# naman1618/Distributed-Inference-with-PyTorch-and-LiteLLM

Hardware: AMD Instinct MI355X
Metric: fine-tune tokens/sec (whole node) Llama-3.1-70B DDP at 1/2/4/8 MI355X (higher is better)
Workload: dtype bf16; 1 GPU; model=Llama-3.1-70B, global_batch=2, seq_len=2048, parallelism=dp1, finetune=lora r=16 alpha=32.0 on q,k,v,o,gate,up,down; frozen bf16 base, micro_batch=2, grad_accum=1, activation_checkpointing=False, optimizer=fused AdamW (HIP), grad clip 1.0, grad_reduce_dtype=bf16

## Files before the change

csrc/kernels/lora.hip:

```cpp
#include "bindings.h"
#include "common.h"
#include <stdlib.h>
#include <string.h>

namespace mx {

namespace {

typedef __bf16 lbf16x8_t __attribute__((ext_vector_type(8)));
typedef __attribute__((address_space(1))) const void* lgptr_t;
typedef __attribute__((address_space(3))) void* llptr_t;

__device__ __forceinline__ f32x4 lmfma(const u16x8& a, const u16x8& b, const f32x4& c) {
  return __builtin_amdgcn_mfma_f32_16x16x32_bf16(__builtin_bit_cast(lbf16x8_t, a), __builtin_bit_cast(lbf16x8_t, b),
                                                 c, 0, 0, 0);
}

constexpr int kRS = 68;
constexpr int kMaxTiles = 16384;

__device__ unsigned int g_xwt_cnt[kMaxTiles];
__device__ unsigned int g_xtg_cnt[kMaxTiles];

__device__ __forceinline__ bool arrive_last(unsigned int* cnt, int S, int* s_flag) {
  __threadfence();
  __syncthreads();
  if (threadIdx.x == 0) {
    const unsigned prev = atomicAdd(cnt, 1u);
    *s_flag = prev == (unsigned)(S - 1);
    if (*s_flag) *cnt = 0u;
  }
  __syncthreads();
  const bool last = *s_flag;
  if (last) __threadfence();
  return last;
}

__device__ __forceinline__ void st4_sc1(float* p, const float4& v) {
  __hip_atomic_store(p + 0, v.x, __ATOMIC_RELAXED, __HIP_MEMORY_SCOPE_AGENT);
  __hip_atomic_store(p + 1, v.y, __ATOMIC_RELAXED, __HIP_MEMORY_SCOPE_AGENT);
  __hip_atomic_store(p + 2, v.z, __ATOMIC_RELAXED, __HIP_MEMORY_SCOPE_AGENT);
  __hip_atomic_store(p + 3, v.w, __ATOMIC_RELAXED, __HIP_MEMORY_SCOPE_AGENT);
}
__device__ __forceinline__ float4 ld4_sc1(const float* p) {
  float* q = const_cast<float*>(p);
  return float4{__hip_atomic_load(q + 0, __ATOMIC_RELAXED, __HIP_MEMORY_SCOPE_AGENT),
                __hip_atomic_load(q + 1, __ATOMIC_RELAXED, __HIP_MEMORY_SCOPE_AGENT),
                __hip_atomic_load(q + 2, __ATOMIC_RELAXED, __HIP_MEMORY_SCOPE_AGENT),
                __hip_atomic_load(q + 3, __ATOMIC_RELAXED, __HIP_MEMORY_SCOPE_AGENT)};
}
__device__ __forceinline__ bool arrive_last_sc1(unsigned int* cnt, int S, int* s_flag) {
  asm volatile("s_waitcnt vmcnt(0)" ::: "memory");
  __syncthreads();
  if (threadIdx.x == 0) {
    const unsigned prev = __hip_atomic_fetch_add(cnt, 1u, __ATOMIC_RELAXED, __HIP_MEMORY_SCOPE_AGENT);
    const int last = prev == (unsigned)(S - 1);
    if (last) __hip_atomic_store(cnt, 0u, __ATOMIC_RELAXED, __HIP_MEMORY_SCOPE_AGENT);
    *s_flag = last;
  }
  __syncthreads();
  return *s_flag;
}

}

__global__ void __launch_bounds__(256, 1) lora_xwt_kernel(const uint16_t* __restrict__ X, int64_t ldx,
                                                          const uint16_t* __restrict__ V, int64_t ldv,
                                                          uint16_t* __restrict__ out, int64_t ldo,
                                                          float* __restrict__ ws, int M, int K, int S, float alpha,
                                                          int fused_red) {
  __shared__ __attribute__((aligned(16))) float red[4][64 * kRS];
  __shared__ int s_last;
  const int mtiles = M >> 6, mt = blockIdx.x, split = blockIdx.y;
  const int tid = threadIdx.x, lane = tid & 63, c = lane & 15, g = lane >> 4;
  const int w = __builtin_amdgcn_readfirstlane(tid >> 6);
  const int nb = K >> 6, nw = S * 4, gw = split * 4 + w;
  const int b0 = (int)((int64_t)gw * nb / nw), b1 = (int)((int64_t)(gw + 1) * nb / nw);
  const uint16_t* xp = X + (int64_t)(mt * 64 + c) * ldx + 16 * g;
  const uint16_t* vp = V + (int64_t)c * ldv + 16 * g;
  const int64_t xrb = 16 * ldx, vcb = 16 * ldv;

  f32x4 acc[4][4];
#pragma unroll
  for (int i = 0; i < 4; ++i)
// ... 155 lines not shown
#pragma unroll
    for (int j = 0; j < 4; ++j)
#pragma unroll
      for (int e = 0; e < 4; ++e) rw[(16 * i + 4 * g + e) * kRS + 16 * j + c] = acc[i][j][e];
  __syncthreads();
  float4 v[4];
#pragma unroll
  for (int q = 0; q < 4; ++q) {
    const int e4 = tid + 256 * q, row = e4 >> 4, col = (e4 & 15) * 4;
    float4 s = *reinterpret_cast<const float4*>(reinterpret_cast<const float*>(smem) + row * kRS + col);
#pragma unroll
    for (int ww = 1; ww < 4; ++ww) {
      const float4 t = *reinterpret_cast<const float4*>(reinterpret_cast<const float*>(smem + ww * WREG) +
                                                        row * kRS + col);
      s.x += t.x, s.y += t.y, s.z += t.z, s.w += t.w;
    }
    v[q] = s;
  }
  if (S > 1) {
    float* wp = ws + ((int64_t)split * mtiles + mt) * 4096;
    if (!fused_red) {
#pragma unroll
      for (int q = 0; q < 4; ++q) reinterpret_cast<float4*>(wp)[tid + 256 * q] = v[q];
      return;
    }
#pragma unroll
    for (int q = 0; q < 4; ++q) st4_sc1(wp + 4 * (tid + 256 * q), v[q]);
    if (!arrive_last_sc1(&g_xwt_cnt[mt], S, s_last)) return;
#pragma unroll
    for (int q = 0; q < 4; ++q) {
      float4 s = ld4_sc1(ws + (int64_t)mt * 4096 + 4 * (tid + 256 * q));
      for (int sp = 1; sp < S; ++sp) {
        const float4 t = ld4_sc1(ws + ((int64_t)sp * mtiles + mt) * 4096 + 4 * (tid + 256 * q));
        s.x += t.x, s.y += t.y, s.z += t.z, s.w += t.w;
      }
      v[q] = s;
    }
  }
#pragma unroll
  for (int q = 0; q < 4; ++q) {
    const int e4 = tid + 256 * q, row = e4 >> 4, col = (e4 & 15) * 4;
    uint2 o;
    o.x = pack_bf16x2(alpha * v[q].x, alpha * v[q].y);
    o.y = pack_bf16x2(alpha * v[q].z, alpha * v[q].w);
    *reinterpret_cast<uint2*>(out + (int64_t)(mt * 64 + row) * ldo + col) = o;
  }
}

__global__ void __launch_bounds__(256) lora_xwt_reduce_kernel(const float* __restrict__ ws, int S, int mtiles,
                                                              uint16_t* __restrict__ out, int64_t ldo, float alpha,
                                                              int qpw) {
  const int per = 4 / qpw;
  const int mt = blockIdx.x / per, tid = threadIdx.x;
  for (int q = (blockIdx.x % per) * qpw; q < (blockIdx.x % per + 1) * qpw; ++q) {
    const int e4 = tid + 256 * q, row = e4 >> 4, col = (e4 & 15) * 4;
    float4 s = reinterpret_cast<const float4*>(ws + (int64_t)mt * 4096)[e4];
    for (int sp = 1; sp < S; ++sp) {
      const float4 t = reinterpret_cast<const float4*>(ws + ((int64_t)sp * mtiles + mt) * 4096)[e4];
      s.x += t.x, s.y += t.y, s.z += t.z, s.w += t.w;
    }
    uint2 o;
    o.x = pack_bf16x2(alpha * s.x, alpha * s.y);
    o.y = pack_bf16x2(alpha * s.z, alpha * s.w);
    *reinterpret_cast<uint2*>(out + (int64_t)(mt * 64 + row) * ldo + col) = o;
  }
}

struct XtgProb {
  const uint16_t* X;
  const uint16_t* G;
  uint16_t* out;
  int64_t ldx, ldg, os_n, os_j;
  int Nx, jb0, JB, tile0;
};
constexpr int kMaxProb = 8;
struct XtgArgs {
  XtgProb p[kMaxProb];
  int np, T, S, ntiles;
  float alpha;
  int accumulate;
  int fused_red;
  int narrow3;
  int wt;
};

__device__ __forceinline__ int xsw(int row) { return (((row >> 1) & 1) << 2) | (((row >> 2) & 1) << 1); }

__global__ void __launch_bounds__(256, 1) lora_xtg_kernel(const XtgArgs a, float* __restrict__ ws) {
  constexpr int XB = 8192, STG = 16384, WREG = 2 * STG;
  __shared__ __attribute__((aligned(16))) char smem[4 * WREG];
  __shared__ int s_last;
  const int tid = threadIdx.x, lane = tid & 63, c = lane & 15, g = lane >> 4;
  const int w = __builtin_amdgcn_readfirstlane(tid >> 6);
  const int tile = a.wt ? blockIdx.x * 4 + w : blockIdx.x, split = blockIdx.y;
  if (a.wt && tile >= a.ntiles) return;
  XtgProb P = a.p[0];
#pragma unroll
  for (int i = 1; i < kMaxProb; ++i)
    if (i < a.np && tile >= a.p[i].tile0) P = a.p[i];
  const int n0 = (tile - P.tile0) * 64;
  const bool wide = P.JB > 1;
  const int JB = P.JB;
  const int qq = c >> 2, pp = c & 3;
  const int nblk = a.T >> 6, nw = a.wt ? a.S : a.S * 4, gw = a.wt ? split : split * 4 + w;
  const int b0 = (int)((int64_t)gw * nblk / nw), b1 = (int)((int64_t)(gw + 1) * nblk / nw);
  char* wreg = smem + w * WREG;
  const uint32_t wbase = lds_addr(wreg);

  const int xrow = lane >> 3, xch = (lane & 7) ^ xsw(lane >> 3);
  const uint16_t* xsrc = P.X + (int64_t)xrow * P.ldx + n0 + 8 * xch;
  const uint16_t* gsrc = wide ? P.G + (int64_t)xrow * P.ldg + 16 * P.jb0 + 8 * xch
                              : P.G + (int64_t)(lane >> 1) * P.ldg + 16 * P.jb0 + 8 * (lane & 1);
  auto issue = [&](int b, int s) {
    const int64_t t0 = (int64_t)b * 64;
    char* xs = wreg + s * STG;
#pragma unroll
    for (int q = 0; q < 8; ++q)
      __builtin_amdgcn_global_load_lds((lgptr_t)(xsrc + (t0 + 8 * q) * P.ldx), (llptr_t)(xs + q * 1024), 16, 0, 0);
    if (wide) {
#pragma unroll
      for (int q = 0; q < 8; ++q)
        __builtin_amdgcn_global_load_lds((lgptr_t)(gsrc + (t0 + 8 * q) * P.ldg), (llptr_t)(xs + XB + q * 1024), 16, 0,
                                         0);
    } else {
#pragma unroll
      for (int q = 0; q < 2; ++q)
        __builtin_amdgcn_global_load_lds((lgptr_t)(gsrc + (t0 + 32 * q) * P.ldg), (llptr_t)(xs + XB + q * 1024), 16,
                                         0, 0);
    }
  };
  const int fl = xsw(4 * g + qq);
  uint32_t xb[4];
#pragma unroll
  for (int i = 0; i < 4; ++i) xb[i] = wbase + (4 * g + qq) * 128 + 16 * ((2 * i + (pp >> 1)) ^ fl) + 8 * (pp & 1);
  const uint32_t gnb = wbase + XB + (4 * g + qq) * 32 + 8 * pp;

  f32x4 acc[4][4];
#pragma unroll
  for (int i = 0; i < 4; ++i)
#pragma unroll
    for (int j = 0; j < 4; ++j) acc[i][j] = f32x4{0.f, 0.f, 0.f, 0.f};

  auto block = [&](auto SC, int b) {
    constexpr int s = decltype(SC)::value;
    if (b + 1 < b1) {
      if (wide) asm volatile("s_waitcnt vmcnt(16)" ::: "memory");
      else asm volatile("s_waitcnt vmcnt(10)" ::: "memory");
    } else {
      asm volatile("s_waitcnt vmcnt(0)" ::: "memory");
    }
    u16x4 xr[2][2][4], gr[2][2][4];
#pragma unroll
    for (int ks = 0; ks < 2; ++ks)
#pragma unroll
      for (int h = 0; h < 2; ++h) {
#pragma unroll
        for (int i = 0; i < 4; ++i) xr[ks][h][i] = trd_off(xb[i], s * STG + (32 * ks + 16 * h) * 128);
        if (wide) {
#pragma unroll
          for (int j = 0; j < 4; ++j)
            if (j < JB) gr[ks][h][j] = trd_off(xb[j], s * STG + XB + (32 * ks + 16 * h) * 128);
        } else {
          gr[ks][h][0] = trd_off(gnb, s * STG + (32 * ks + 16 * h) * 32);
        }
      }
    lds_wait();
#pragma unroll
    for (int ks = 0; ks < 2; ++ks)
#pragma unroll
      for (int h = 0; h < 2; ++h) {
#pragma unroll
        for (int i = 0; i < 4; ++i) pin(xr[ks][h][i]);
#pragma unroll
        for (int j = 0; j < 4; ++j)
          if (j < JB) pin(gr[ks][h][j]);
      }
    if (b + 2 < b1) issue(b + 2, s);
#pragma unroll
    for (int ks = 0; ks < 2; ++ks) {
#pragma unroll
      for (int j = 0; j < 4; ++j) {
        if (j >= JB) continue;
        const u16x8 bf = u16x8{gr[ks][0][j][0], gr[ks][0][j][1], gr[ks][0][j][2], gr[ks][0][j][3],
                               gr[ks][1][j][0], gr[ks][1][j][1], gr[ks][1][j][2], gr[ks][1][j][3]};
#pragma unroll
        for (int i = 0; i < 4; ++i) {
          const u16x8 af = u16x8{xr[ks][0][i][0], xr[ks][0][i][1], xr[ks][0][i][2], xr[ks][0][i][3],
                                 xr[ks][1][i][0], xr[ks][1][i][1], xr[ks][1][i][2], xr[ks][1][i][3]};
          acc[i][j] = lmfma(af, bf, acc[i][j]);
        }
      }
    }
  };
  if (wide || !a.narrow3) {
    if (b0 < b1) issue(b0, 0);
    if (b0 + 1 < b1) issue(b0 + 1, 1);
    for (int b = b0; b < b1; b += 2) {
      block(std::integral_constant<int, 0>{}, b);
      if (b + 1 < b1) block(std::integral_constant<int, 1>{}, b + 1);
    }
  } else {
    constexpr int STN = XB + 2048;
    auto issue3 = [&](int b, int st) {
      const int64_t t0 = (int64_t)b * 64;
      char* xs = wreg + st * STN;
#pragma unroll
      for (int q = 0; q < 8; ++q)
        __builtin_amdgcn_global_load_lds((lgptr_t)(xsrc + (t0 + 8 * q) * P.ldx), (llptr_t)(xs + q * 1024), 16, 0, 0);
#pragma unroll
      for (int q = 0; q < 2; ++q)
        __builtin_amdgcn_global_load_lds((lgptr_t)(gsrc + (t0 + 32 * q) * P.ldg), (llptr_t)(xs + XB + q * 1024), 16,
                                         0, 0);
    };
    auto block3 = [&](auto SC, int b) {
      constexpr int st = decltype(SC)::value;
      if (b + 2 < b1) asm volatile("s_waitcnt vmcnt(20)" ::: "memory");
      else if (b + 1 < b1) asm volatile("s_waitcnt vmcnt(10)" ::: "memory");
      else asm volatile("s_waitcnt vmcnt(0)" ::: "memory");
      u16x4 xr[2][2][4], gr[2][2];
#pragma unroll
      for (int ks = 0; ks < 2; ++ks)
#pragma unroll
        for (int h = 0; h < 2; ++h) {
#pragma unroll
          for (int i = 0; i < 4; ++i) xr[ks][h][i] = trd_off(xb[i], st * STN + (32 * ks + 16 * h) * 128);
          gr[ks][h] = trd_off(gnb, st * STN + (32 * ks + 16 * h) * 32);
        }
      lds_wait();
#pragma unroll
      for (int ks = 0; ks < 2; ++ks)
#pragma unroll
        for (int h = 0; h < 2; ++h) {
#pragma unroll
          for (int i = 0; i < 4; ++i) pin(xr[ks][h][i]);
          pin(gr[ks][h]);
        }
      if (b + 3 < b1) issue3(b + 3, st);
#pragma unroll
      for (int ks = 0; ks < 2; ++ks) {
        const u16x8 bf = u16x8{gr[ks][0][0], gr[ks][0][1], gr[ks][0][2], gr[ks][0][3],
                               gr[ks][1][0], gr[ks][1][1], gr[ks][1][2], gr[ks][1][3]};
#pragma unroll
        for (int i = 0; i < 4; ++i) {
          const u16x8 af = u16x8{xr[ks][0][i][0], xr[ks][0][i][1], xr[ks][0][i][2], xr[ks][0][i][3],
                                 xr[ks][1][i][0], xr[ks][1][i][1], xr[ks][1][i][2], xr[ks][1][i][3]};
          acc[i][0] = lmfma(af, bf, acc[i][0]);
        }
      }
    };
    if (b0 < b1) issue3(b0, 0);
    if (b0 + 1 < b1) issue3(b0 + 1, 1);
    if (b0 + 2 < b1) issue3(b0 + 2, 2);
    for (int b = b0; b < b1; b += 3) {
      block3(std::integral_constant<int, 0>{}, b);
      if (b + 1 < b1) block3(std::integral_constant<int, 1>{}, b + 1);
      if (b + 2 < b1) block3(std::integral_constant<int, 2>{}, b + 2);
    }
  }
  float* rw = reinterpret_cast<float*>(wreg);
#pragma unroll
  for (int i = 0; i < 4; ++i)
#pragma unroll
    for (int j = 0; j < 4; ++j) {
      if (j >= JB) continue;
#pragma unroll
      for (int e = 0; e < 4; ++e) rw[(16 * i + 4 * g + e) * kRS + 16 * j + c] = acc[i][j][e];
    }
  if (a.wt) {
    asm volatile("s_waitcnt lgkmcnt(0)" ::: "memory");
    __builtin_amdgcn_wave_barrier();
    const int J = 16 * JB, nel = 64 * J;
    const bool jfast = P.os_j == 1;
    for (int e = lane; e < nel; e += 64) {
      const int n = jfast ? e / J : (e & 63), j = jfast ? e % J : (e >> 6);
      uint16_t* o = P.out + (int64_t)(n0 + n) * P.os_n + (int64_t)j * P.os_j;
      const float r = a.alpha * rw[n * kRS + j] + (a.accumulate ? bf2f(*o) : 0.f);
      *o = f2bf(r);
    }
    return;
  }
  __syncthreads();
  const int J = 16 * JB, nel = 64 * J;
  const bool jfast = P.os_j == 1;
  float v[16];
#pragma unroll
  for (int q = 0; q < 16; ++q) {
    const int e = tid + 256 * q;
    v[q] = 0.f;
    if (e < nel) {
      const int n = jfast ? e / J : (e & 63), j = jfast ? e % J : (e >> 6);
      float s = 0.f;
#pragma unroll
      for (int ww = 0; ww < 4; ++ww) s += reinterpret_cast<const float*>(smem + ww * WREG)[n * kRS + j];
      v[q] = s;
    }
  }
  if (a.S > 1) {
    float* wp = ws + ((int64_t)split * a.ntiles + tile) * 4096;
    if (!a.fused_red) {
#pragma unroll
      for (int q = 0; q < 16; ++q)
        if (tid + 256 * q < nel) wp[tid + 256 * q] = v[q];
      return;
    }
#pragma unroll
    for (int q = 0; q < 16; ++q)
      if (tid + 256 * q < nel) __hip_atomic_store(wp + tid + 256 * q, v[q], __ATOMIC_RELAXED, __HIP_MEMORY_SCOPE_AGENT);
    if (!arrive_last_sc1(&g_xtg_cnt[tile], a.S, &s_last)) return;
#pragma unroll
    for (int q = 0; q < 16; ++q) {
      const int e = tid + 256 * q;
      if (e < nel) {
        float s = __hip_atomic_load(ws + (int64_t)tile * 4096 + e, __ATOMIC_RELAXED, __HIP_MEMORY_SCOPE_AGENT);
        for (int sp = 1; sp < a.S; ++sp)
          s += __hip_atomic_load(ws + ((int64_t)sp * a.ntiles + tile) * 4096 + e, __ATOMIC_RELAXED,
                                 __HIP_MEMORY_SCOPE_AGENT);
        v[q] = s;
      }
    }
  }
#pragma unroll
  for (int q = 0; q < 16; ++q) {
    const int e = tid + 256 * q;
    if (e < nel) {
      const int n = jfast ? e / J : (e & 63), j = jfast ? e % J : (e >> 6);
      uint16_t* o = P.out + (int64_t)(n0 + n) * P.os_n + (int64_t)j * P.os_j;
      const float r = a.alpha * v[q] + (a.accumulate ? bf2f(*o) : 0.f);
      *o = f2bf(r);
    }
  }
}

__global__ void __launch_bounds__(256) lora_xtg_reduce_kernel(const XtgArgs a, const float* __restrict__ ws) {
  const int tile = blockIdx.x, tid = threadIdx.x;
  XtgProb P = a.p[0];
#pragma unroll
  for (int i = 1; i < kMaxProb; ++i)
    if (i < a.np && tile >= a.p[i].tile0) P = a.p[i];
  const int n0 = (tile - P.tile0) * 64, J = 16 * P.JB, nel = 64 * J;
  const bool jfast = P.os_j == 1;
  for (int e = tid; e < nel; e += 256) {
    float s = ws[(int64_t)tile * 4096 + e];
    for (int sp = 1; sp < a.S; ++sp) s += ws[((int64_t)sp * a.ntiles + tile) * 4096 + e];
    const int n = jfast ? e / J : (e & 63), j = jfast ? e % J : (e >> 6);
    uint16_t* o = P.out + (int64_t)(n0 + n) * P.os_n + (int64_t)j * P.os_j;
    *o = f2bf(a.alpha * s + (a.accumulate ? bf2f(*o) : 0.f));
  }
}

constexpr int kSlRow = 136;

__device__ __forceinline__ float sl_sigmoid(float x) { return __builtin_amdgcn_rcpf(1.f + __expf(-x)); }

template <bool BWD, int NRB, int RBW>
__global__ void __launch_bounds__(256) swiglu_lora_kernel(const uint16_t* __restrict__ gu,
                                                          const uint16_t* __restrict__ dm, uint16_t* __restrict__ out,
                                                          int64_t ldo, const uint16_t* __restrict__ V, int64_t ldv,
                                                          float* __restrict__ ws, int F, int CS) {
  constexpr int NP = BWD ? 2 : 1;
  constexpr int NC = 16 * NRB;
  __shared__ __attribute__((aligned(16))) uint16_t img[2][NP][RBW][16 * kSlRow];
  __shared__ __attribute__((aligned(16))) float red[4][16][NC + 4];
  const int rg = blockIdx.x, split = blockIdx.y, tid = threadIdx.x;
  const int lane = tid & 63, w = tid >> 6, r = lane & 15, gq = lane >> 4;
  const int row = tid >> 4, ch = tid & 15;
  const int tiles = F >> 7;
  const int t0 = (int)((int64_t)split * tiles / CS), t1 = (int)((int64_t)(split + 1) * tiles / CS);
  const int64_t tok = (int64_t)rg * 16 * RBW + row;
  const uint16_t* grow = gu + tok * (2 * (int64_t)F) + 8 * ch;
  const uint16_t* drow = dm + tok * (int64_t)F + 8 * ch;
  uint16_t* orow = out + tok * ldo + 8 * ch;
  const int64_t gstep = 16 * (2 * (int64_t)F), dstep = 16 * (int64_t)F, ostep = 16 * ldo;
  const uint16_t* vrow = V + (int64_t)r * ldv + 32 * w + 8 * gq;
  const int wofs = row * kSlRow + 8 * ch, rofs = r * kSlRow + 32 * w + 8 * gq;

  f32x4 acc[RBW][NRB];
#pragma unroll
  for (int i = 0; i < RBW; ++i)
#pragma unroll
    for (int b = 0; b < NRB; ++b) acc[i][b] = f32x4{0.f, 0.f, 0.f, 0.f};

  u16x8 g[RBW], u[RBW], d[RBW], vf[NP][NRB];
  auto vload = [&](int t) {
#pragma unroll
    for (int p = 0; p < NP; ++p)
#pragma unroll
      for (int b = 0; b < NRB; ++b)
        vf[p][b] = *reinterpret_cast<const u16x8*>(vrow + (int64_t)(16 * b) * ldv + p * F + (t << 7));
  };
  auto load = [&](int t, u16x8(&g_)[RBW], u16x8(&u_)[RBW], u16x8(&d_)[RBW]) {
    const int c = t << 7;
#pragma unroll
    for (int i = 0; i < RBW; ++i) {
      g_[i] = *reinterpret_cast<const u16x8*>(grow + i * gstep + c);
      u_[i] = *reinterpret_cast<const u16x8*>(grow + i * gstep + F + c);
      if (BWD) d_[i] = *reinterpret_cast<const u16x8*>(drow + i * dstep + c);
    }
  };
  if (t0 < t1) {
    load(t0, g, u, d);
    vload(t0);
  }
  for (int t = t0; t < t1; ++t) {
    const int c = t << 7, buf = (t - t0) & 1;
    u16x8 gn[RBW], un[RBW], dn[RBW];
    load(t + 1 < t1 ? t + 1 : t, gn, un, dn);
#pragma unroll
    for (int i = 0; i < RBW; ++i) {
      u16x8 o0, o1;
      if (!BWD) {
#pragma unroll
        for (int j = 0; j < 8; ++j) {
          const float gf = bf2f(g[i][j]);
          o0[j] = f2bf(gf * sl_sigmoid(gf) * bf2f(u[i][j]));
        }
        *reinterpret_cast<u16x8*>(orow + i * ostep + c) = o0;
        *reinterpret_cast<u16x8*>(&img[buf][0][i][wofs]) = o0;
      } else {
#pragma unroll
        for (int j = 0; j < 8; ++j) {
          const float gf = bf2f(g[i][j]), uf = bf2f(u[i][j]), df = bf2f(d[i][j]);
          float dg, du;
          swiglu_grad(df, gf, uf, dg, du);
          o0[j] = f2bf(dg);
          o1[j] = f2bf(du);
        }
        *reinterpret_cast<u16x8*>(orow + i * ostep + c) = o0;
        *reinterpret_cast<u16x8*>(orow + i * ostep + F + c) = o1;
        *reinterpret_cast<u16x8*>(&img[buf][0][i][wofs]) = o0;
// ... 103 lines not shown
    for (int b = 0; b < NRB; ++b)
#pragma unroll
      for (int e = 0; e < 4; ++e) red[w][4 * gq + e][16 * b + r] = acc[i][b][e];
    __syncthreads();
    float* wp = ws + ((int64_t)split * (gridDim.x * RBW) + rg * RBW + i) * (16 * NC);
    for (int k = tid; k < 16 * NC; k += 256) {
      const int rr = k / NC, cc = k % NC;
      wp[k] = ((red[0][rr][cc] + red[1][rr][cc]) + red[2][rr][cc]) + red[3][rr][cc];
    }
  }
}

}

using namespace mx;

static int lora_env(const char* name, int dflt);

static int swiglu_lora_rbw(int T) {
  int rbw = lora_env("MXLLM_SWIGLU_LORA_RBW", 2);
  rbw = rbw >= 4 ? 4 : (rbw >= 2 ? 2 : 1);
  while (rbw > 1 && (T / 16) % rbw) rbw >>= 1;
  return rbw;
}

static int swiglu_lora_splits(int T, int F) {
  const int tiles = F / 128, rbs = T / (16 * swiglu_lora_rbw(T));
  int cs = lora_env("MXLLM_SWIGLU_LORA_CS", 0);
  if (cs <= 0) cs = (512 + rbs - 1) / rbs;
  cs = cs < 1 ? 1 : cs;
  cs = cs > tiles ? tiles : cs;
  return cs > 32 ? 32 : cs;
}

extern "C" int64_t mx_swiglu_lora_ws(int T, int F, int nrb) {
  if (T <= 0 || F < 128) return 0;
  return (int64_t)swiglu_lora_splits(T, F) * T * 16 * nrb;
}

extern "C" int mx_swiglu_lora(int bwd, const uint16_t* gu, const uint16_t* dm, uint16_t* out, int64_t ldo,
                              const uint16_t* V, int64_t ldv, int nrb, int pad, float alpha, float* ws, int T, int F,
                              hipStream_t stream) {
  if (T <= 0) return 0;
  if (T % 16 || F % 128 || nrb < 1 || nrb > 4 || pad < 16 * nrb || pad % 8 || ldo % 8 || ldv % 8 ||
      ldo < (bwd ? 2 * (int64_t)F : F) + pad || ((uintptr_t)gu | (uintptr_t)out | (uintptr_t)V) % 16 ||
      (bwd && (!dm || (uintptr_t)dm % 16)))
    return (int)hipErrorInvalidValue;
  const int CS = swiglu_lora_splits(T, F), RBW = swiglu_lora_rbw(T);
  const dim3 grid(T / (16 * RBW), CS);
#define MX_SL_R(B, N, R) swiglu_lora_kernel<B, N, R><<<grid, 256, 0, stream>>>(gu, dm, out, ldo, V, ldv, ws, F, CS)
#define MX_SL(B, N)                                 \
  do {                                              \
    if (RBW == 4) MX_SL_R(B, N, 4);                 \
    else if (RBW == 2) MX_SL_R(B, N, 2);            \
    else MX_SL_R(B, N, 1);                          \
  } while (0)
  if (bwd) {
    switch (nrb) { case 1: MX_SL(true, 1); break; case 2: MX_SL(true, 2); break;
                   case 3: MX_SL(true, 3); break; default: MX_SL(true, 4); break; }
  } else {
    switch (nrb) { case 1: MX_SL(false, 1); break; case 2: MX_SL(false, 2); break;
                   case 3: MX_SL(false, 3); break; default: MX_SL(false, 4); break; }
  }
#undef MX_SL
#undef MX_SL_R
  swiglu_lora_reduce_kernel<<<T / 16, 256, 0, stream>>>(ws, CS, 16 * nrb, pad, out + (bwd ? 2 * (int64_t)F : F), ldo,
                                                        alpha);
  return (int)hipGetLastError();
}

static int lora_env(const char* name, int dflt) {
  const char* v = getenv(name);
  return v && *v ? atoi(v) : dflt;
}
static int lora_splits(int tiles, int blocks, int smax) {
  if (tiles <= 0) return 1;
  const int target = lora_env("MXLLM_LORA_WGS", 256);
  int S = (target + tiles - 1) / tiles;
  S = S < 1 ? 1 : (S > smax ? smax : S);
  while (S > 1 && blocks / (4 * S) < 2) --S;
  return S;
}

static bool xtg_wave_tiles(int ntiles) {
  return lora_env("MXLLM_LORA_XTG_WT", 1) == 1 && ntiles >= lora_env("MXLLM_LORA_XTG_WT_MIN", 1024);
}

static int xwt_mode() {
  const char* kv = getenv("MXLLM_LORA_XWT");
  if (kv && !strcmp(kv, "reg")) return 2;
  if (kv && !strcmp(kv, "tile")) return 0;
  return 1;
}
static bool xwt_tile_ok(const void* X, int64_t ldx, const void* V, int64_t ldv, int M, int K, int rows) {
  return xwt_mode() == 0 && M % 16 == 0 && K % 128 == 0 && rows > 0 && rows <= 64 && ldx % 8 == 0 &&
         ldv % 8 == 0 && (uintptr_t)X % 16 == 0 && (uintptr_t)V % 16 == 0;
}
static int xwt_rbw(int M) { return M % 64 == 0 ? 4 : (M % 32 == 0 ? 2 : 1); }
static int xwt_tile_splits(int M, int K) {
  const int groups = M / (16 * xwt_rbw(M)), tiles = K / 128;
  int cs = lora_env("MXLLM_LORA_XWT_CS", 0);
  if (cs <= 0) cs = (512 + groups - 1) / groups;
  cs = cs < 1 ? 1 : cs;
  return cs > tiles ? tiles : cs;
}

extern "C" int64_t mx_lora_xwt_ws(int M, int K, int rows) {
  const int S = M >= 64 && K >= 64 ? lora_splits(M / 64, K / 64, 16) : 1;
  const int64_t dma = S > 1 ? (int64_t)S * (M / 64) * 4096 : 0;
  if (rows > 0 && rows <= 64 && M % 16 == 0 && K % 128 == 0 && xwt_mode() == 0) {
    const int64_t tile = (int64_t)xwt_tile_splits(M, K) * M * 16 * ((rows + 15) / 16);
    return tile > dma ? tile : dma;
  }
  return dma;
}
extern "C" int64_t mx_lora_xtg_ws(int ntiles, int T) {
  if (xtg_wave_tiles(ntiles)) return 0;
  const int S = lora_splits(ntiles, T / 64, 8);
  return S > 1 ? (int64_t)S * ntiles * 4096 : 0;
}

extern "C" int mx_lora_xwt(const uint16_t* X, int64_t ldx, const uint16_t* V, int64_t ldv, int Vrows, uint16_t* out,
                           int64_t ldo, float* ws, int M, int K, float alpha, int rows, hipStream_t stream) {
  if (M <= 0) return 0;
  if (xwt_tile_ok(X, ldx, V, ldv, M, K, rows) && rows <= Vrows && ldo % 4 == 0) {
    const int nrb = (rows + 15) / 16, rbw = xwt_rbw(M), CS = xwt_tile_splits(M, K);
    const dim3 grid(M / (16 * rbw), CS);
#define MX_XT(N, R) lora_xwt_tile_kernel<N, R><<<grid, 256, 0, stream>>>(X, ldx, V, ldv, ws, K, CS)
#define MX_XT_N(R)                                  \
  switch (nrb) {                                    \
    case 1: MX_XT(1, R); break;                     \
    case 2: MX_XT(2, R); break;                     \
    case 3: MX_XT(3, R); break;                     \
    default: MX_XT(4, R); break;                    \
  }
    if (rbw == 4) { MX_XT_N(4) } else if (rbw == 2) { MX_XT_N(2) } else { MX_XT_N(1) }
#undef MX_XT_N
#undef MX_XT
    swiglu_lora_reduce_kernel<<<M / 16, 256, 0, stream>>>(ws, CS, 16 * nrb, Vrows, out, ldo, alpha);
    return (int)hipGetLastError();
  }
  if (M % 64 || K % 64 || Vrows % 64 || M / 64 > kMaxTiles) return (int)hipErrorInvalidValue;
  const int mtiles = M / 64, S = lora_splits(mtiles, K / 64, 16);
  const int fused = lora_env("MXLLM_LORA_FUSED_RED", 0);
  const bool lds = xwt_mode() != 2 && ((uintptr_t)X % 16 == 0) && ((uintptr_t)V % 16 == 0) && ldx % 8 == 0 &&
                   ldv % 8 == 0;
  for (int c0 = 0; c0 < Vrows; c0 += 64) {
    if (lds)
      lora_xwt_lds_kernel<<<dim3(mtiles, S), 256, 0, stream>>>(X, ldx, V + (int64_t)c0 * ldv, ldv, out + c0, ldo, ws,
                                                               M, K, S, alpha, fused);
    else
      lora_xwt_kernel<<<dim3(mtiles, S), 256, 0, stream>>>(X, ldx, V + (int64_t)c0 * ldv, ldv, out + c0, ldo, ws, M,
                                                           K, S, alpha, fused);
    if (S > 1 && !fused) {
      const int qpw = lora_env("MXLLM_LORA_XWT_RED_ROWS", 16) >= 64 ? 4 : 1;
      lora_xwt_reduce_kernel<<<(4 / qpw) * mtiles, 256, 0, stream>>>(ws, S, mtiles, out + c0, ldo, alpha, qpw);
    }
  }
  return (int)hipGetLastError();
}

extern "C" int mx_lora_xtg(const int64_t* desc, int np, int T, float alpha, int accumulate, float* ws,
                           hipStream_t stream) {
  if (np <= 0 || np > kMaxProb || T % 64) return (int)hipErrorInvalidValue;
  if (T == 0) return 0;
  XtgArgs a{};
  int ntiles = 0;
  for (int i = 0; i < np; ++i) {
    const int64_t* d = desc + i * 10;
    XtgProb& p = a.p[i];
    p.X = reinterpret_cast<const uint16_t*>(d[0]);
    p.G = reinterpret_cast<const uint16_t*>(d[1]);
    p.out = reinterpret_cast<uint16_t*>(d[2]);
    p.ldx = d[3], p.ldg = d[4], p.os_n = d[5], p.os_j = d[6];
    p.Nx = (int)d[7], p.jb0 = (int)d[8], p.JB = (int)d[9];
    if (p.Nx <= 0 || p.Nx % 64 || p.JB < 1 || p.JB > 4) return (int)hipErrorInvalidValue;
    p.tile0 = ntiles;
    ntiles += p.Nx / 64;
  }
  if (ntiles > kMaxTiles) return (int)hipErrorInvalidValue;
  a.np = np, a.T = T, a.ntiles = ntiles, a.alpha = alpha;
  a.wt = xtg_wave_tiles(ntiles);
  a.S = a.wt ? 1 : lora_splits(ntiles, T / 64, 8);
  a.accumulate = accumulate;
  a.fused_red = a.wt ? 0 : lora_env("MXLLM_LORA_FUSED_RED", 0);
  a.narrow3 = lora_env("MXLLM_LORA_XTG_STAGES", 3) == 3;
  lora_xtg_kernel<<<dim3(a.wt ? (ntiles + 3) / 4 : ntiles, a.S), 256, 0, stream>>>(a, ws);
  if (a.S > 1 && !a.fused_red) lora_xtg_reduce_kernel<<<ntiles, 256, 0, stream>>>(a, ws);
  return (int)hipGetLastError();
}
```

Baseline: 4661 tokens/s.

## Stream-K partition LoRA X^T·G wave-tile kernel across fixed workgroup count

Replaces the one-tile-per-wave launch of the LoRA gradient X^T·G kernel with a stream-K style split: a fixed number of workgroups each walk a contiguous range of (tile-group, row-block) units, writing partial tiles to workspace slots that a vectorized reduce kernel then sums. It also lowers the tile-count threshold for taking the wave-tile path, so more shapes use it. The aim is to remove load imbalance and tail waves when the tile count does not divide evenly across CUs. The cost is extra workspace traffic and a second reduce launch whenever a tile group is split across workgroups.

```diff
diff --git a/csrc/kernels/lora.hip b/csrc/kernels/lora.hip
--- a/csrc/kernels/lora.hip
+++ b/csrc/kernels/lora.hip
@@ -1,5 +1,6 @@
 #include "bindings.h"
 #include "common.h"
+#include "lora_xtg_part.h"
 #include <stdlib.h>
 #include <string.h>
 
@@ -321,202 +322,239 @@
   int fused_red;
   int narrow3;
   int wt;
+  int W;
+  int rev;
 };
 
 __device__ __forceinline__ int xsw(int row) { return (((row >> 1) & 1) << 2) | (((row >> 2) & 1) << 1); }
 
+template <bool WT>
 __global__ void __launch_bounds__(256, 1) lora_xtg_kernel(const XtgArgs a, float* __restrict__ ws) {
   constexpr int XB = 8192, STG = 16384, WREG = 2 * STG;
   __shared__ __attribute__((aligned(16))) char smem[4 * WREG];
   __shared__ int s_last;
   const int tid = threadIdx.x, lane = tid & 63, c = lane & 15, g = lane >> 4;
   const int w = __builtin_amdgcn_readfirstlane(tid >> 6);
-  const int tile = a.wt ? blockIdx.x * 4 + w : blockIdx.x, split = blockIdx.y;
-  if (a.wt && tile >= a.ntiles) return;
-  XtgProb P = a.p[0];
-#pragma unroll
-  for (int i = 1; i < kMaxProb; ++i)
-    if (i < a.np && tile >= a.p[i].tile0) P = a.p[i];
-  const int n0 = (tile - P.tile0) * 64;
-  const bool wide = P.JB > 1;
-  const int JB = P.JB;
+  const int split = blockIdx.y, nblk = a.T >> 6;
   const int qq = c >> 2, pp = c & 3;
-  const int nblk = a.T >> 6, nw = a.wt ? a.S : a.S * 4, gw = a.wt ? split : split * 4 + w;
-  const int b0 = (int)((int64_t)gw * nblk / nw), b1 = (int)((int64_t)(gw + 1) * nblk / nw);
   char* wreg = smem + w * WREG;
   const uint32_t wbase = lds_addr(wreg);
-
-  const int xrow = lane >> 3, xch = (lane & 7) ^ xsw(lane >> 3);
-  const uint16_t* xsrc = P.X + (int64_t)xrow * P.ldx + n0 + 8 * xch;
-  const uint16_t* gsrc = wide ? P.G + (int64_t)xrow * P.ldg + 16 * P.jb0 + 8 * xch
-                              : P.G + (int64_t)(lane >> 1) * P.ldg + 16 * P.jb0 + 8 * (lane & 1);
-  auto issue = [&](int b, int s) {
-    const int64_t t0 = (int64_t)b * 64;
-    char* xs = wreg + s * STG;
-#pragma unroll
-    for (int q = 0; q < 8; ++q)
-      __builtin_amdgcn_global_load_lds((lgptr_t)(xsrc + (t0 + 8 * q) * P.ldx), (llptr_t)(xs + q * 1024), 16, 0, 0);
-    if (wide) {
+  const XtgPart part = xtg_part(a.ntiles, nblk, a.W);
+  int64_t u = WT ? xtg_run_begin(part, blockIdx.x) : 0;
+  const int64_t uend = WT ? xtg_run_begin(part, blockIdx.x + 1) : 0;
+  XtgProb P;
+  int tile, n0, JB;
+  for (;;) {
+    int b0, b1;
+    if (WT) {
+      const int grp = (int)xtg_div(u, nblk);
+      b0 = (int)(u - (int64_t)grp * nblk);
+      b1 = uend - u < nblk - b0 ? b0 + (int)(uend - u) : nblk;
+      u += b1 - b0;
+      tile = 4 * grp + w;
+      if (tile >= a.ntiles) {
+        if (u >= uend) return;
+        continue;
+      }
+    } else {
+      const int nw = a.S * 4, gw = split * 4 + w;
+      tile = blockIdx.x;
+      b0 = (int)((int64_t)gw * nblk / nw), b1 = (int)((int64_t)(gw + 1) * nblk / nw);
+    }
+    P = a.p[0];
+#pragma unroll
+    for (int i = 1; i < kMaxProb; ++i)
+      if (i < a.np && tile >= a.p[i].tile0) P = a.p[i];
+    n0 = (tile - P.tile0) * 64;
+    const bool wide = P.JB > 1;
+    JB = P.JB;
+    const int bflip = WT && a.rev ? b0 + b1 - 1 : -1;
+    auto rowblk = [&](int b) { return bflip >= 0 ? bflip - b : b; };
+
+    const int xrow = lane >> 3, xch = (lane & 7) ^ xsw(lane >> 3);
+    const uint16_t* xsrc = P.X + (int64_t)xrow * P.ldx + n0 + 8 * xch;
+    const uint16_t* gsrc = wide ? P.G + (int64_t)xrow * P.ldg + 16 * P.jb0 + 8 * xch
+                                : P.G + (int64_t)(lane >> 1) * P.ldg + 16 * P.jb0 + 8 * (lane & 1);
+    auto issue = [&](int b, int s) {
+      const int64_t t0 = (int64_t)rowblk(b) * 64;
+      char* xs = wreg + s * STG;
 #pragma unroll
       for (int q = 0; q < 8; ++q)
-        __builtin_amdgcn_global_load_lds((lgptr_t)(gsrc + (t0 + 8 * q) * P.ldg), (llptr_t)(xs + XB + q * 1024), 16, 0,
-                                         0);
+        __builtin_amdgcn_global_load_lds((lgptr_t)(xsrc + (t0 + 8 * q) * P.ldx), (llptr_t)(xs + q * 1024), 16, 0, 0);
+      if (wide) {
+#pragma unroll
+        for (int q = 0; q < 8; ++q)
+          __builtin_amdgcn_global_load_lds((lgptr_t)(gsrc + (t0 + 8 * q) * P.ldg), (llptr_t)(xs + XB + q * 1024), 16, 0,
+                                           0);
+      } else {
+#pragma unroll
+        for (int q = 0; q < 2; ++q)
+          __builtin_amdgcn_global_load_lds((lgptr_t)(gsrc + (t0 + 32 * q) * P.ldg), (llptr_t)(xs + XB + q * 1024), 16,
+                                           0, 0);
+      }
+    };
+    const int fl = xsw(4 * g + qq);
+    uint32_t xb[4];
+#pragma unroll
+    for (int i = 0; i < 4; ++i) xb[i] = wbase + (4 * g + qq) * 128 + 16 * ((2 * i + (pp >> 1)) ^ fl) + 8 * (pp & 1);
+    const uint32_t gnb = wbase + XB + (4 * g + qq) * 32 + 8 * pp;
+
+    f32x4 acc[4][4];
+#pragma unroll
+    for (int i = 0; i < 4; ++i)
+#pragma unroll
+      for (int j = 0; j < 4; ++j) acc[i][j] = f32x4{0.f, 0.f, 0.f, 0.f};
+
+    auto block = [&](auto SC, int b) {
+      constexpr int s = decltype(SC)::value;
+      if (b + 1 < b1) {
+        if (wide) asm volatile("s_waitcnt vmcnt(16)" ::: "memory");
+        else asm volatile("s_waitcnt vmcnt(10)" ::: "memory");
+      } else {
+        asm volatile("s_waitcnt vmcnt(0)" ::: "memory");
+      }
+      u16x4 xr[2][2][4], gr[2][2][4];
+#pragma unroll
+      for (int ks = 0; ks < 2; ++ks)
+#pragma unroll
+        for (int h = 0; h < 2; ++h) {
+#pragma unroll
+          for (int i = 0; i < 4; ++i) xr[ks][h][i] = trd_off(xb[i], s * STG + (32 * ks + 16 * h) * 128);
+          if (wide) {
+#pragma unroll
+            for (int j = 0; j < 4; ++j)
+              if (j < JB) gr[ks][h][j] = trd_off(xb[j], s * STG + XB + (32 * ks + 16 * h) * 128);
+          } else {
+            gr[ks][h][0] = trd_off(gnb, s * STG + (32 * ks + 16 * h) * 32);
+          }
+        }
+      lds_wait();
+#pragma unroll
+      for (int ks = 0; ks < 2; ++ks)
+#pragma unroll
+        for (int h = 0; h < 2; ++h) {
+#pragma unroll
+          for (int i = 0; i < 4; ++i) pin(xr[ks][h][i]);
+#pragma unroll
+          for (int j = 0; j < 4; ++j)
+            if (j < JB) pin(gr[ks][h][j]);
+        }
+      if (b + 2 < b1) issue(b + 2, s);
+#pragma unroll
+      for (int ks = 0; ks < 2; ++ks) {
+#pragma unroll
+        for (int j = 0; j < 4; ++j) {
+          if (j >= JB) continue;
+          const u16x8 bf = u16x8{gr[ks][0][j][0], gr[ks][0][j][1], gr[ks][0][j][2], gr[ks][0][j][3],
+                                 gr[ks][1][j][0], gr[ks][1][j][1], gr[ks][1][j][2], gr[ks][1][j][3]};
+#pragma unroll
+          for (int i = 0; i < 4; ++i) {
+            const u16x8 af = u16x8{xr[ks][0][i][0], xr[ks][0][i][1], xr[ks][0][i][2], xr[ks][0][i][3],
+                                   xr[ks][1][i][0], xr[ks][1][i][1], xr[ks][1][i][2], xr[ks][1][i][3]};
+            acc[i][j] = lmfma(af, bf, acc[i][j]);
+          }
+        }
+      }
+    };
+    if (wide || !a.narrow3) {
+      if (b0 < b1) issue(b0, 0);
+      if (b0 + 1 < b1) issue(b0 + 1, 1);
+      for (int b = b0; b < b1; b += 2) {
+        block(std::integral_constant<int, 0>{}, b);
+        if (b + 1 < b1) block(std::integral_constant<int, 1>{}, b + 1);
+      }
     } else {
-#pragma unroll
-      for (int q = 0; q < 2; ++q)
-        __builtin_amdgcn_global_load_lds((lgptr_t)(gsrc + (t0 + 32 * q) * P.ldg), (llptr_t)(xs + XB + q * 1024), 16,
-                                         0, 0);
-    }
-  };
-  const int fl = xsw(4 * g + qq);
-  uint32_t xb[4];
-#pragma unroll
-  for (int i = 0; i < 4; ++i) xb[i] = wbase + (4 * g + qq) * 128 + 16 * ((2 * i + (pp >> 1)) ^ fl) + 8 * (pp & 1);
-  const uint32_t gnb = wbase + XB + (4 * g + qq) * 32 + 8 * pp;
-
-  f32x4 acc[4][4];
-#pragma unroll
-  for (int i = 0; i < 4; ++i)
-#pragma unroll
-    for (int j = 0; j < 4; ++j) acc[i][j] = f32x4{0.f, 0.f, 0.f, 0.f};
-
-  auto block = [&](auto SC, int b) {
-    constexpr int s = decltype(SC)::value;
-    if (b + 1 < b1) {
-      if (wide) asm volatile("s_waitcnt vmcnt(16)" ::: "memory");
-      else asm volatile("s_waitcnt vmcnt(10)" ::: "memory");
-    } else {
-      asm volatile("s_waitcnt vmcnt(0)" ::: "memory");
-    }
-    u16x4 xr[2][2][4], gr[2][2][4];
-#pragma unroll
-    for (int ks = 0; ks < 2; ++ks)
-#pragma unroll
-      for (int h = 0; h < 2; ++h) {
-#pragma unroll
-        for (int i = 0; i < 4; ++i) xr[ks][h][i] = trd_off(xb[i], s * STG + (32 * ks + 16 * h) * 128);
-        if (wide) {
-#pragma unroll
-          for (int j = 0; j < 4; ++j)
-            if (j < JB) gr[ks][h][j] = trd_off(xb[j], s * STG + XB + (32 * ks + 16 * h) * 128);
-        } else {
-          gr[ks][h][0] = trd_off(gnb, s * STG + (32 * ks + 16 * h) * 32);
+      constexpr int STN = XB + 2048;
+      auto issue3 = [&](int b, int st) {
+        const int64_t t0 = (int64_t)rowblk(b) * 64;
+        char* xs = wreg + st * STN;
+#pragma unroll
+        for (int q = 0; q < 8; ++q)
+          __builtin_amdgcn_global_load_lds((lgptr_t)(xsrc + (t0 + 8 * q) * P.ldx), (llptr_t)(xs + q * 1024), 16, 0, 0);
+#pragma unroll
+        for (int q = 0; q < 2; ++q)
+          __builtin_amdgcn_global_load_lds((lgptr_t)(gsrc + (t0 + 32 * q) * P.ldg), (llptr_t)(xs + XB + q * 1024), 16,
+                                           0, 0);
+      };
+      auto block3 = [&](auto SC, int b) {
+        constexpr int st = decltype(SC)::value;
+        if (b + 2 < b1) asm volatile("s_waitcnt vmcnt(20)" ::: "memory");
+        else if (b + 1 < b1) asm volatile("s_waitcnt vmcnt(10)" ::: "memory");
+        else asm volatile("s_waitcnt vmcnt(0)" ::: "memory");
+        u16x4 xr[2][2][4], gr[2][2];
+#pragma unroll
+        for (int ks = 0; ks < 2; ++ks)
+#pragma unroll
+          for (int h = 0; h < 2; ++h) {
+#pragma unroll
+            for (int i = 0; i < 4; ++i) xr[ks][h][i] = trd_off(xb[i], st * STN + (32 * ks + 16 * h) * 128);
+            gr[ks][h] = trd_off(gnb, st * STN + (32 * ks + 16 * h) * 32);
+          }
+        lds_wait();
+#pragma unroll
+        for (int ks = 0; ks < 2; ++ks)
+#pragma unroll
+          for (int h = 0; h < 2; ++h) {
+#pragma unroll
+            for (int i = 0; i < 4; ++i) pin(xr[ks][h][i]);
+            pin(gr[ks][h]);
+          }
+        if (b + 3 < b1) issue3(b + 3, st);
+#pragma unroll
+        for (int ks = 0; ks < 2; ++ks) {
+          const u16x8 bf = u16x8{gr[ks][0][0], gr[ks][0][1], gr[ks][0][2], gr[ks][0][3],
+                                 gr[ks][1][0], gr[ks][1][1], gr[ks][1][2], gr[ks][1][3]};
+#pragma unroll
+          for (int i = 0; i < 4; ++i) {
+            const u16x8 af = u16x8{xr[ks][0][i][0], xr[ks][0][i][1], xr[ks][0][i][2], xr[ks][0][i][3],
+                                   xr[ks][1][i][0], xr[ks][1][i][1], xr[ks][1][i][2], xr[ks][1][i][3]};
+            acc[i][0] = lmfma(af, bf, acc[i][0]);
+          }
         }
-      }
-    lds_wait();
-#pragma unroll
-    for (int ks = 0; ks < 2; ++ks)
-#pragma unroll
-      for (int h = 0; h < 2; ++h) {
-#pragma unroll
-        for (int i = 0; i < 4; ++i) pin(xr[ks][h][i]);
-#pragma unroll
-        for (int j = 0; j < 4; ++j)
-          if (j < JB) pin(gr[ks][h][j]);
-      }
-    if (b + 2 < b1) issue(b + 2, s);
-#pragma unroll
-    for (int ks = 0; ks < 2; ++ks) {
+      };
+      if (b0 < b1) issue3(b0, 0);
+      if (b0 + 1 < b1) issue3(b0 + 1, 1);
+      if (b0 + 2 < b1) issue3(b0 + 2, 2);
+      for (int b = b0; b < b1; b += 3) {
+        block3(std::integral_constant<int, 0>{}, b);
+        if (b + 1 < b1) block3(std::integral_constant<int, 1>{}, b + 1);
+        if (b + 2 < b1) block3(std::integral_constant<int, 2>{}, b + 2);
+      }
+    }
+    float* rw = reinterpret_cast<float*>(wreg);
+#pragma unroll
+    for (int i = 0; i < 4; ++i)
 #pragma unroll
       for (int j = 0; j < 4; ++j) {
         if (j >= JB) continue;
-        const u16x8 bf = u16x8{gr[ks][0][j][0], gr[ks][0][j][1], gr[ks][0][j][2], gr[ks][0][j][3],
-                               gr[ks][1][j][0], gr[ks][1][j][1], gr[ks][1][j][2], gr[ks][1][j][3]};
-#pragma unroll
-        for (int i = 0; i < 4; ++i) {
-          const u16x8 af = u16x8{xr[ks][0][i][0], xr[ks][0][i][1], xr[ks][0][i][2], xr[ks][0][i][3],
-                                 xr[ks][1][i][0], xr[ks][1][i][1], xr[ks][1][i][2], xr[ks][1][i][3]};
-          acc[i][j] = lmfma(af, bf, acc[i][j]);
+#pragma unroll
+        for (int e = 0; e < 4; ++e) rw[(16 * i + 4 * g + e) * kRS + 16 * j + c] = acc[i][j][e];
+      }
+    if (WT) {
+      asm volatile("s_waitcnt lgkmcnt(0)" ::: "memory");
+      __builtin_amdgcn_wave_barrier();
+      const int J = 16 * JB, nel = 64 * J;
+      const bool jfast = P.os_j == 1;
+      if (b1 - b0 == nblk) {
+        for (int e = lane; e < nel; e += 64) {
+          const int n = jfast ? e / J : (e & 63), j = jfast ? e % J : (e >> 6);
+          uint16_t* o = P.out + (int64_t)(n0 + n) * P.os_n + (int64_t)j * P.os_j;
+          const float r = a.alpha * rw[n * kRS + j] + (a.accumulate ? bf2f(*o) : 0.f);
+          *o = f2bf(r);
         }
-      }
-    }
-  };
-  if (wide || !a.narrow3) {
-    if (b0 < b1) issue(b0, 0);
-    if (b0 + 1 < b1) issue(b0 + 1, 1);
-    for (int b = b0; b < b1; b += 2) {
-      block(std::integral_constant<int, 0>{}, b);
-      if (b + 1 < b1) block(std::integral_constant<int, 1>{}, b + 1);
-    }
-  } else {
-    constexpr int STN = XB + 2048;
-    auto issue3 = [&](int b, int st) {
-      const int64_t t0 = (int64_t)b * 64;
-      char* xs = wreg + st * STN;
-#pragma unroll
-      for (int q = 0; q < 8; ++q)
-        __builtin_amdgcn_global_load_lds((lgptr_t)(xsrc + (t0 + 8 * q) * P.ldx), (llptr_t)(xs + q * 1024), 16, 0, 0);
-#pragma unroll
-      for (int q = 0; q < 2; ++q)
-        __builtin_amdgcn_global_load_lds((lgptr_t)(gsrc + (t0 + 32 * q) * P.ldg), (llptr_t)(xs + XB + q * 1024), 16,
-                                         0, 0);
-    };
-    auto block3 = [&](auto SC, int b) {
-      constexpr int st = decltype(SC)::value;
-      if (b + 2 < b1) asm volatile("s_waitcnt vmcnt(20)" ::: "memory");
-      else if (b + 1 < b1) asm volatile("s_waitcnt vmcnt(10)" ::: "memory");
-      else asm volatile("s_waitcnt vmcnt(0)" ::: "memory");
-      u16x4 xr[2][2][4], gr[2][2];
-#pragma unroll
-      for (int ks = 0; ks < 2; ++ks)
-#pragma unroll
-        for (int h = 0; h < 2; ++h) {
-#pragma unroll
-          for (int i = 0; i < 4; ++i) xr[ks][h][i] = trd_off(xb[i], st * STN + (32 * ks + 16 * h) * 128);
-          gr[ks][h] = trd_off(gnb, st * STN + (32 * ks + 16 * h) * 32);
+      } else {
+        float* wp = ws + xtg_slot(part, tile, (int)blockIdx.x - xtg_first(part, tile >> 2)) * kXtgSlotFloats;
+        for (int e = lane; e < nel; e += 64) {
+          const int n = jfast ? e / J : (e & 63), j = jfast ? e % J : (e >> 6);
+          wp[e] = rw[n * kRS + j];
         }
-      lds_wait();
-#pragma unroll
-      for (int ks = 0; ks < 2; ++ks)
-#pragma unroll
-        for (int h = 0; h < 2; ++h) {
-#pragma unroll
-          for (int i = 0; i < 4; ++i) pin(xr[ks][h][i]);
-          pin(gr[ks][h]);
-        }
-      if (b + 3 < b1) issue3(b + 3, st);
-#pragma unroll
-      for (int ks = 0; ks < 2; ++ks) {
-        const u16x8 bf = u16x8{gr[ks][0][0], gr[ks][0][1], gr[ks][0][2], gr[ks][0][3],
-                               gr[ks][1][0], gr[ks][1][1], gr[ks][1][2], gr[ks][1][3]};
-#pragma unroll
-        for (int i = 0; i < 4; ++i) {
-          const u16x8 af = u16x8{xr[ks][0][i][0], xr[ks][0][i][1], xr[ks][0][i][2], xr[ks][0][i][3],
-                                 xr[ks][1][i][0], xr[ks][1][i][1], xr[ks][1][i][2], xr[ks][1][i][3]};
-          acc[i][0] = lmfma(af, bf, acc[i][0]);
-        }
-      }
-    };
-    if (b0 < b1) issue3(b0, 0);
-    if (b0 + 1 < b1) issue3(b0 + 1, 1);
-    if (b0 + 2 < b1) issue3(b0 + 2, 2);
-    for (int b = b0; b < b1; b += 3) {
-      block3(std::integral_constant<int, 0>{}, b);
-      if (b + 1 < b1) block3(std::integral_constant<int, 1>{}, b + 1);
-      if (b + 2 < b1) block3(std::integral_constant<int, 2>{}, b + 2);
-    }
-  }
-  float* rw = reinterpret_cast<float*>(wreg);
-#pragma unroll
-  for (int i = 0; i < 4; ++i)
-#pragma unroll
-    for (int j = 0; j < 4; ++j) {
-      if (j >= JB) continue;
-#pragma unroll
-      for (int e = 0; e < 4; ++e) rw[(16 * i + 4 * g + e) * kRS + 16 * j + c] = acc[i][j][e];
-    }
-  if (a.wt) {
-    asm volatile("s_waitcnt lgkmcnt(0)" ::: "memory");
-    __builtin_amdgcn_wave_barrier();
-    const int J = 16 * JB, nel = 64 * J;
-    const bool jfast = P.os_j == 1;
-    for (int e = lane; e < nel; e += 64) {
-      const int n = jfast ? e / J : (e & 63), j = jfast ? e % J : (e >> 6);
-      uint16_t* o = P.out + (int64_t)(n0 + n) * P.os_n + (int64_t)j * P.os_j;
-      const float r = a.alpha * rw[n * kRS + j] + (a.accumulate ? bf2f(*o) : 0.f);
-      *o = f2bf(r);
-    }
-    return;
+      }
+      if (u >= uend) return;
+      asm volatile("s_waitcnt vmcnt(0) lgkmcnt(0)" ::: "memory");
+      __builtin_amdgcn_wave_barrier();
+      continue;
+    }
+    break;
   }
   __syncthreads();
   const int J = 16 * JB, nel = 64 * J;
@@ -572,18 +610,37 @@
 
 __global__ void __launch_bounds__(256) lora_xtg_reduce_kernel(const XtgArgs a, const float* __restrict__ ws) {
   const int tile = blockIdx.x, tid = threadIdx.x;
+  const XtgPart part = xtg_part(a.ntiles, a.T >> 6, a.W);
+  const int nparts = a.wt ? xtg_nparts(part, tile >> 2) : a.S;
+  if (a.wt && nparts == 1) return;
+  const int64_t slot0 = a.wt ? xtg_slot(part, tile, 0) : tile, sstep = a.wt ? 4 : a.ntiles;
   XtgProb P = a.p[0];
 #pragma unroll
   for (int i = 1; i < kMaxProb; ++i)
     if (i < a.np && tile >= a.p[i].tile0) P = a.p[i];
   const int n0 = (tile - P.tile0) * 64, J = 16 * P.JB, nel = 64 * J;
   const bool jfast = P.os_j == 1;
-  for (int e = tid; e < nel; e += 256) {
-    float s = ws[(int64_t)tile * 4096 + e];
-    for (int sp = 1; sp < a.S; ++sp) s += ws[((int64_t)sp * a.ntiles + tile) * 4096 + e];
-    const int n = jfast ? e / J : (e & 63), j = jfast ? e % J : (e >> 6);
-    uint16_t* o = P.out + (int64_t)(n0 + n) * P.os_n + (int64_t)j * P.os_j;
-    *o = f2bf(a.alpha * s + (a.accumulate ? bf2f(*o) : 0.f));
+  const float* w0 = ws + slot0 * 4096;
+  const int64_t wstep = sstep * 4096;
+  for (int e4 = tid; 4 * e4 < nel; e4 += 256) {
+    float4 s = reinterpret_cast<const float4*>(w0)[e4];
+    for (int sp = 1; sp < nparts; sp += 8) {
+      float4 t[8];
+#pragma unroll
+      for (int k = 0; k < 8; ++k)
+        if (sp + k < nparts) t[k] = reinterpret_cast<const float4*>(w0 + (sp + k) * wstep)[e4];
+#pragma unroll
+      for (int k = 0; k < 8; ++k)
+        if (sp + k < nparts) s.x += t[k].x, s.y += t[k].y, s.z += t[k].z, s.w += t[k].w;
+    }
+    const float v[4] = {s.x, s.y, s.z, s.w};
+#pragma unroll
+    for (int k = 0; k < 4; ++k) {
+      const int e = 4 * e4 + k;
+      const int n = jfast ? e / J : (e & 63), j = jfast ? e % J : (e >> 6);
+      uint16_t* o = P.out + (int64_t)(n0 + n) * P.os_n + (int64_t)j * P.os_j;
+      *o = f2bf(a.alpha * v[k] + (a.accumulate ? bf2f(*o) : 0.f));
+    }
   }
 }
 
@@ -853,9 +910,11 @@
   return S;
 }
 
+constexpr int kXtgWtMinDefault = 576;
 static bool xtg_wave_tiles(int ntiles) {
-  return lora_env("MXLLM_LORA_XTG_WT", 1) == 1 && ntiles >= lora_env("MXLLM_LORA_XTG_WT_MIN", 1024);
-}
+  return lora_env("MXLLM_LORA_XTG_WT", 1) == 1 && ntiles >= lora_env("MXLLM_LORA_XTG_WT_MIN", kXtgWtMinDefault);
+}
+static XtgPart xtg_wt_part(int ntiles, int T) { return xtg_part(ntiles, T / 64, lora_env("MXLLM_LORA_WGS", 256)); }
 
 static int xwt_mode() {
   const char* kv = getenv("MXLLM_LORA_XWT");
@@ -886,7 +945,8 @@
   return dma;
 }
 extern "C" int64_t mx_lora_xtg_ws(int ntiles, int T) {
-  if (xtg_wave_tiles(ntiles)) return 0;
+  if (ntiles <= 0 || T < 64) return 0;
+  if (xtg_wave_tiles(ntiles)) return xtg_ws_floats(xtg_wt_part(ntiles, T));
   const int S = lora_splits(ntiles, T / 64, 8);
   return S > 1 ? (int64_t)S * ntiles * 4096 : 0;
 }
@@ -956,7 +1016,15 @@
   a.accumulate = accumulate;
   a.fused_red = a.wt ? 0 : lora_env("MXLLM_LORA_FUSED_RED", 0);
   a.narrow3 = lora_env("MXLLM_LORA_XTG_STAGES", 3) == 3;
-  lora_xtg_kernel<<<dim3(a.wt ? (ntiles + 3) / 4 : ntiles, a.S), 256, 0, stream>>>(a, ws);
+  if (a.wt) {
+    const XtgPart part = xtg_wt_part(ntiles, T);
+    a.W = part.W;
+    a.rev = lora_env("MXLLM_LORA_XTG_REV", 0) == 1;
+    lora_xtg_kernel<true><<<a.W, 256, 0, stream>>>(a, ws);
+    if (xtg_any_partial(part)) lora_xtg_reduce_kernel<<<ntiles, 256, 0, stream>>>(a, ws);
+    return (int)hipGetLastError();
+  }
+  lora_xtg_kernel<false><<<dim3(ntiles, a.S), 256, 0, stream>>>(a, ws);
   if (a.S > 1 && !a.fused_red) lora_xtg_reduce_kernel<<<ntiles, 256, 0, stream>>>(a, ws);
   return (int)hipGetLastError();
 }
diff --git a/csrc/kernels/lora_xtg_part.h b/csrc/kernels/lora_xtg_part.h
--- /dev/null
+++ b/csrc/kernels/lora_xtg_part.h
@@ -0,0 +1,59 @@
+#pragma once
+#include <stdint.h>
+
+#if defined(__HIPCC__) || defined(__CUDACC__)
+#define MX_XTG_HD __host__ __device__ inline
+#else
+#define MX_XTG_HD inline
+#endif
+
+namespace mx {
+
+constexpr int kXtgSlotFloats = 4096;
+
+struct XtgPart {
+  int ntiles, nblk, W, ngroups;
+  int64_t U;
+};
+
+constexpr int kXtgMaxW = 65536;
+
+MX_XTG_HD XtgPart xtg_part(int ntiles, int nblk, int wgs) {
+  XtgPart p;
+  p.ntiles = ntiles, p.nblk = nblk;
+  p.ngroups = (ntiles + 3) / 4;
+  p.U = (int64_t)p.ngroups * nblk;
+  wgs = wgs < 1 ? 1 : (wgs > kXtgMaxW ? kXtgMaxW : wgs);
+  p.W = (int)(wgs < p.U ? wgs : p.U);
+  return p;
+}
+
+MX_XTG_HD int64_t xtg_div(int64_t a, int64_t b) {
+  return ((uint64_t)(a | b) >> 32) == 0 ? (int64_t)((uint32_t)a / (uint32_t)b) : a / b;
+}
+
+MX_XTG_HD int64_t xtg_run_begin(const XtgPart& p, int i) { return xtg_div((int64_t)i * p.U, p.W); }
+
+MX_XTG_HD int xtg_owner(const XtgPart& p, int64_t u) { return (int)xtg_div((u + 1) * p.W - 1, p.U); }
+
+MX_XTG_HD int xtg_first(const XtgPart& p, int g) { return xtg_owner(p, (int64_t)g * p.nblk); }
+MX_XTG_HD int xtg_nparts(const XtgPart& p, int g) {
+  return xtg_owner(p, (int64_t)(g + 1) * p.nblk - 1) - xtg_first(p, g) + 1;
+}
+
+MX_XTG_HD int64_t xtg_slot(const XtgPart& p, int tile, int pos) {
+  const int g = tile >> 2;
+  return ((int64_t)xtg_first(p, g) + g + pos) * 4 + (tile & 3);
+}
+
+MX_XTG_HD bool xtg_any_partial(const XtgPart& p) {
+  for (int g = 0; g < p.ngroups; ++g)
+    if (xtg_nparts(p, g) > 1) return true;
+  return false;
+}
+
+MX_XTG_HD int64_t xtg_ws_floats(const XtgPart& p) {
+  return xtg_any_partial(p) ? ((int64_t)p.W + p.ngroups - 1) * 4 * kXtgSlotFloats : 0;
+}
+
+}
```

New measurement: 4659 tokens/s, median of 2. No clear change (-0.0%).
